# shurizzle/cake

Hardware: AMD Instinct MI355X
Metric: decode_tokens_per_sec (higher is better)
Workload: dtype bf16; 1 GPU; model=Llama-3-8B, global_batch=1, seq_len=1097, prompt_len=32, parallelism=single, decode=greedy, repeat_penalty 1.10 last_n 128

## Files before the change

### cake_amd/csrc/kernels/gemv_kernel.h

```cpp
#pragma once
#include <type_traits>

#include "common.h"

namespace cake {

constexpr int kGemvThreads = 256;
constexpr int kGemvWaves = kGemvThreads / 64;
constexpr int kGemvMaxBlocks = 1024;

typedef float f32x2_t __attribute__((ext_vector_type(2)));

struct GemvTune { int U, PF, MB; };
enum GemvKind { kQkv = 0, kSwiglu = 1, kX16 = 2, kNormF32 = 3, kX16S = 4, kNumKinds = 5 };
extern GemvTune g_tune[4][kNumKinds];


template <class T>
__device__ __forceinline__ const T* pick3(const T* q, const T* k, const T* v, int kind) {
  const ptrdiff_t dk = k - q, dv = v - q;
  return q + (kind == 0 ? 0 : (kind == 1 ? dk : dv));
}

struct PlainRows {
  struct Rows { const uint4 *a, *b; };
  struct Chunk { uint4 a, b; };
  template <bool NT> static __device__ __forceinline__ Chunk load(const Rows& r, int c) {
    if constexpr (NT) return {ld_nt16(r.a + c), ld_nt16(r.b + c)};
    else return {r.a[c], r.b[c]};
  }
  template <int LOG2> static int prefetch_if_filled(int pf, int K) {
    return (K >> LOG2) >= 64 * pf ? pf : 0;
  }
};

template <int DT, bool XF32>
__device__ __forceinline__ void load_x8(const void* xs, int chunk, float* o) {
  if constexpr (XF32) {
    const float4* p = reinterpret_cast<const float4*>(xs) + chunk * 2;
    const float4 a = p[0], b = p[1];
    o[0] = a.x; o[1] = a.y; o[2] = a.z; o[3] = a.w;
    o[4] = b.x; o[5] = b.y; o[6] = b.z; o[7] = b.w;
  } else {
    unpack8<DT>(reinterpret_cast<const uint4*>(xs)[chunk], o);
  }
}

struct W16 : PlainRows {
  static constexpr int kFmt = 0, kKinds = kNumKinds, kLog2 = 3, kPad32 = 1, kPad16 = 1;
  static constexpr int kU[3] = {2, 4, 8}, kPF[2] = {8, 4};
  static constexpr bool kStrict = false, kRowScale = false;
  static __device__ __forceinline__ int perm32(int i) { return i; }
  static __device__ __forceinline__ int perm16(int i) { return i; }
  static int prefetch(int pf, int K) { return prefetch_if_filled<kLog2>(pf, K); }
  using Acc = float;
  static __device__ __forceinline__ Acc zero() { return 0.f; }
  static __device__ __forceinline__ float total(Acc a) { return a; }
  struct Mat { const uint16_t* w; };
  static __device__ __forceinline__ Mat pick(const Mat& q, const Mat& k, const Mat& v, int kind) {
    return {pick3(q.w, k.w, v.w, kind)};
  }
  static __device__ __forceinline__ Rows rows(const Mat& ma, size_t ra, const Mat& mb, size_t rb,
                                              int K) {
    return {reinterpret_cast<const uint4*>(ma.w + ra * K),
            reinterpret_cast<const uint4*>(mb.w + rb * K)};
  }
  template <int DT, bool XF32>
  static __device__ __forceinline__ void fma(const void* xs, int chunk, const Chunk& v, Acc& acc_a,
                                             Acc& acc_b) {
    float xv[8], fa[8], fb[8];
    load_x8<DT, XF32>(xs, chunk, xv);
    unpack8<DT>(v.a, fa);
    unpack8<DT>(v.b, fb);
#pragma unroll
    for (int e = 0; e < 8; ++e) {
      acc_a = fmaf(fa[e], xv[e], acc_a);
      acc_b = fmaf(fb[e], xv[e], acc_b);
    }
  }
};

template <class F, class = void> struct HasRawRows : std::false_type {};
template <class F>
struct HasRawRows<F, std::void_t<decltype(F::kRawRows)>> : std::bool_constant<F::kRawRows> {};

template <class F, class = void> struct Bf16Only : std::false_type {};
template <class F>
struct Bf16Only<F, std::void_t<decltype(F::kBf16Only)>> : std::bool_constant<F::kBf16Only> {};

template <class F, int U, class = void> struct X16Waves : std::integral_constant<int, 1> {};
template <class F, int U>
struct X16Waves<F, U, std::void_t<decltype(F::x16_waves(U))>>
    : std::integral_constant<int, F::x16_waves(U)> {};

template <class F>
__device__ __forceinline__ float row_scale(const typename F::Mat& m, size_t row) {
  if constexpr (F::kRowScale) return m.scale[row];
  else return 1.f;
}
template <class F>
__device__ __forceinline__ float descale(float d, bool first, float s0, const typename F::Mat& m,
                                         size_t row) {
  if constexpr (F::kRowScale) return d * (first ? s0 : m.scale[row]);
  else return d;
}


template <class F, int DT>
__device__ __forceinline__ void stage_rmsnorm(const float* __restrict__ x,
                                              const uint16_t* __restrict__ w,
                                              float eps, int K, float* xs) {
  __shared__ float red[16];
  float ss = 0.f;
  for (int i = threadIdx.x * 4; i < K; i += kGemvThreads * 4) {
    const float4 v = *reinterpret_cast<const float4*>(x + i);
    *reinterpret_cast<float4*>(xs + F::perm32(i)) = v;
    ss += v.x * v.x + v.y * v.y + v.z * v.z + v.w * v.w;
  }
  ss = block_sum(ss, red);
  const float r = rsqrtf(ss / (float)K + eps);
  for (int i = threadIdx.x * 4; i < K; i += kGemvThreads * 4) {
    float4 v = *reinterpret_cast<float4*>(xs + F::perm32(i));
    const uint2 wv = *reinterpret_cast<const uint2*>(w + i);
    v.x *= r * to_f32<DT>((uint16_t)(wv.x & 0xffff));
    v.y *= r * to_f32<DT>((uint16_t)(wv.x >> 16));
    v.z *= r * to_f32<DT>((uint16_t)(wv.y & 0xffff));
    v.w *= r * to_f32<DT>((uint16_t)(wv.y >> 16));
    *reinterpret_cast<float4*>(xs + F::perm32(i)) = v;
  }
  __syncthreads();
}

template <class F>
__device__ __forceinline__ void stage_plain16(const uint16_t* __restrict__ x, int K,
                                              uint16_t* xs) {
  for (int i = threadIdx.x * 8; i < K; i += kGemvThreads * 8)
    *reinterpret_cast<uint4*>(xs + F::perm16(i)) = *reinterpret_cast<const uint4*>(x + i);
  __syncthreads();
}

template <class F, int DT, int NX> struct NormPre {
  float4 x[NX];
  uint2 w[NX];
  __device__ __forceinline__ void load(const float* __restrict__ xg, const uint16_t* __restrict__ wg,
                                       int K) {
#pragma unroll
    for (int j = 0; j < NX; ++j) {
      const int i = (j * kGemvThreads + threadIdx.x) * 4;
      x[j] = i < K ? *reinterpret_cast<const float4*>(xg + i) : make_float4(0.f, 0.f, 0.f, 0.f);
      w[j] = i < K ? *reinterpret_cast<const uint2*>(wg + i) : make_uint2(0u, 0u);
    }
  }
  __device__ __forceinline__ void finish(float eps, int K, float* xs) {
    __shared__ float red[16];
    float ss = 0.f;
#pragma unroll
    for (int j = 0; j < NX; ++j) ss += x[j].x * x[j].x + x[j].y * x[j].y + x[j].z * x[j].z + x[j].w * x[j].w;
    ss = block_sum(ss, red);
    const float r = rsqrtf(ss / (float)K + eps);
#pragma unroll
    for (int j = 0; j < NX; ++j) {
      const int i = (j * kGemvThreads + threadIdx.x) * 4;
      float4 v = x[j];
      v.x *= r * to_f32<DT>((uint16_t)(w[j].x & 0xffff));
      v.y *= r * to_f32<DT>((uint16_t)(w[j].x >> 16));
      v.z *= r * to_f32<DT>((uint16_t)(w[j].y & 0xffff));
      v.w *= r * to_f32<DT>((uint16_t)(w[j].y >> 16));
      if (i < K) *reinterpret_cast<float4*>(xs + F::perm32(i)) = v;
    }
    __syncthreads();
  }
};

template <class F, int NX> struct Plain16Pre {
  uint4 v[NX];
  __device__ __forceinline__ void load(const uint16_t* __restrict__ xg, int K) {
#pragma unroll
    for (int j = 0; j < NX; ++j) {
      const int i = (j * kGemvThreads + threadIdx.x) * 8;
      v[j] = i < K ? *reinterpret_cast<const uint4*>(xg + i) : make_uint4(0u, 0u, 0u, 0u);
    }
  }
  __device__ __forceinline__ void finish(int K, uint16_t* xs) {
#pragma unroll
    for (int j = 0; j < NX; ++j) {
      const int i = (j * kGemvThreads + threadIdx.x) * 8;
      if (i < K) *reinterpret_cast<uint4*>(xs + F::perm16(i)) = v[j];
    }
    __syncthreads();
  }
};


template <class F, int DT, bool XF32, int U>
__device__ __forceinline__ void dot_range(const typename F::Rows& r, const void* xs, int nch,
                                          int c_start, typename F::Acc& acc_a,
                                          typename F::Acc& acc_b) {
  const int lane = threadIdx.x & 63;
  const int full = c_start + ((nch - c_start) / (64 * U)) * (64 * U);
  for (int c0 = c_start; c0 < full; c0 += 64 * U) {
    typename F::Chunk v[U];
#pragma unroll
    for (int u = 0; u < U; ++u) v[u] = F::template load<true>(r, c0 + u * 64 + lane);
#pragma unroll
    for (int u = 0; u < U; ++u) F::template fma<DT, XF32>(xs, c0 + u * 64 + lane, v[u], acc_a, acc_b);
  }
  for (int c = full + lane; c < nch; c += 64)
    F::template fma<DT, XF32>(xs, c, F::template load<false>(r, c), acc_a, acc_b);
}

template <class F, int PFC, bool RAW = HasRawRows<F>::value> struct Regs {
  typename F::Chunk c[PFC > 0 ? PFC : 1];
};
template <class F, int PFC> struct Regs<F, PFC, true> {
  typename F::Chunk c[PFC > 0 ? PFC : 1];
  typename F::Rows r;
};

template <class F, int PFC>
__device__ __forceinline__ void prefetch_rows(const typename F::Rows& r, Regs<F, PFC>& g) {
  if constexpr (PFC > 0) {
    const int lane = threadIdx.x & 63;
#pragma unroll
    for (int c = 0; c < PFC; ++c) g.c[c] = F::template load<true>(r, c * 64 + lane);
  }
}

template <class F, int PFC>
__device__ __forceinline__ void keep_rows(const typename F::Rows& r, Regs<F, PFC>& g) {
  if constexpr (HasRawRows<F>::value) g.r = r;
}

template <class F, int DT, bool XF32, int U, int PFC, class Map, class Epi>
__device__ __forceinline__ void run_pairs_raw(const Map& map, const Epi& epi, const void* xs, int K,
                                              int npairs, int p0, int stride,
                                              const Regs<F, PFC>& pre) {
  const int nch = K >> F::kLog2;
  auto raw_dots = [&](const typename F::Rows& r, float& aa, float& ab) {
    dot_range<W16, DT, XF32, 4>(F::raw_rows(r, K), xs, K >> W16::kLog2, 0, aa, ab);
  };
  auto clamped = [&](int q) { return map(q < npairs ? q : npairs - 1); };
  int p = p0;
  typename F::Rows rn;
  if constexpr (PFC > 0) {
    const typename F::Rows r = pre.r;
    rn = clamped(p + stride);
    const int lane = threadIdx.x & 63;
    if (F::is_raw(r)) {
      float aa = 0.f, ab = 0.f;
      raw_dots(r, aa, ab);
      const float sa = wave_sum(aa), sb = wave_sum(ab);
      if (p < npairs) epi(p, sa, sb);
    } else {
      typename F::Acc aa = F::zero(), ab = F::zero();
#pragma unroll
      for (int c = 0; c < PFC; ++c) F::template fma<DT, XF32>(xs, c * 64 + lane, pre.c[c], aa, ab);
      dot_range<F, DT, XF32, U>(r, xs, nch, PFC * 64, aa, ab);
      const float sa = wave_sum(F::total(aa)), sb = wave_sum(F::total(ab));
      if (p < npairs) epi(p, sa, sb);
    }
    p += stride;
  } else {
    rn = clamped(p);
  }
  for (; p < npairs; p += stride) {
    const typename F::Rows r = rn;
    rn = clamped(p + stride);
    if (F::is_raw(r)) {
      float aa = 0.f, ab = 0.f;
      raw_dots(r, aa, ab);
      epi(p, wave_sum(aa), wave_sum(ab));
      continue;
    }
    typename F::Acc aa = F::zero(), ab = F::zero();
    dot_range<F, DT, XF32, U>(r, xs, nch, 0, aa, ab);
    epi(p, wave_sum(F::total(aa)), wave_sum(F::total(ab)));
  }
}

template <class F, int DT, bool XF32, int U, int PFC, class Map, class Epi>
__device__ __forceinline__ void run_pairs(const Map& map, const Epi& epi, const void* xs, int K,
                                          int npairs, int p0, int stride,
                                          const Regs<F, PFC>& pre) {
  if constexpr (HasRawRows<F>::value) {
    run_pairs_raw<F, DT, XF32, U, PFC>(map, epi, xs, K, npairs, p0, stride, pre);
    return;
  }
  const int nch = K >> F::kLog2;
  int p = p0;
  if constexpr (PFC > 0) {
    const typename F::Rows r = map(p < npairs ? p : npairs - 1);
    const int lane = threadIdx.x & 63;
    typename F::Acc aa = F::zero(), ab = F::zero();
#pragma unroll
    for (int c = 0; c < PFC; ++c) F::template fma<DT, XF32>(xs, c * 64 + lane, pre.c[c], aa, ab);
    dot_range<F, DT, XF32, U>(r, xs, nch, PFC * 64, aa, ab);
    const float sa = wave_sum(F::total(aa)), sb = wave_sum(F::total(ab));
    if (p < npairs) epi(p, sa, sb);
    p += stride;
  }
  for (; p < npairs; p += stride) {
    const typename F::Rows r = map(p);
    typename F::Acc aa = F::zero(), ab = F::zero();
    dot_range<F, DT, XF32, U>(r, xs, nch, 0, aa, ab);
    epi(p, wave_sum(F::total(aa)), wave_sum(F::total(ab)));
  }
}

template <class F> struct QkvArgs {
  const float* resid;
  const uint16_t* norm_w;
  float eps;
  typename F::Mat q, k, v;
  int K, nh, nkv, hd;
  const float* inv_freq;
  const int* pos;
  float* q_out;
  uint16_t* kcache;
  uint16_t* vcache;
  int S;
  int kv_fmt;
};

struct QkvPair {
  int kind, head, i;
  size_t ra;
};

__device__ __forceinline__ QkvPair qkv_pair(int p, int half, int nh, int nqk, int hd) {
  const int slot = p / half;
  const bool isq = slot < nh, isk = !isq && slot < nqk;
  QkvPair r;
  r.kind = isq ? 0 : (isk ? 1 : 2);
  r.head = slot - (isq ? 0 : (isk ? nh : nqk));
  r.i = p - slot * half;
  r.ra = (size_t)r.head * hd + r.i;
  return r;
}

template <class F, int DT, int U, int PFC, int NX>
__global__ __launch_bounds__(kGemvThreads) void qkv_rope_kernel(QkvArgs<F> a) {
  extern __shared__ float xs[];
  const int half = a.hd >> 1;
  const int npairs = (a.nh + 2 * a.nkv) * half;
  const int wave = threadIdx.x >> 6, lane = threadIdx.x & 63;
  const int p0 = blockIdx.x * kGemvWaves + wave;
  const int nh = a.nh, nqk = a.nh + a.nkv, hd = a.hd, K = a.K;
  auto map = [&](int p) {
    const QkvPair r = qkv_pair(p, half, nh, nqk, hd);
    const typename F::Mat m = F::pick(a.q, a.k, a.v, r.kind);
    return F::rows(m, r.ra, m, r.ra + half, K);
  };
  Regs<F, PFC> pre;
  NormPre<F, DT, NX> xp;
  const int pc = p0 < npairs ? p0 : npairs - 1;
  const typename F::Rows r0 = map(pc);
  keep_rows<F, PFC>(r0, pre);
  if constexpr (NX > 0) xp.load(a.resid, a.norm_w, a.K);
  __builtin_amdgcn_sched_barrier(0);
  if (NX > 0 || (PFC > 0 && p0 < npairs)) prefetch_rows<F, PFC>(r0, pre);
  const QkvPair rc = qkv_pair(pc, half, nh, nqk, hd);
  const float f0 = a.inv_freq[rc.i];
  const typename F::Mat mc = F::pick(a.q, a.k, a.v, rc.kind);
  const float s0a = row_scale<F>(mc, rc.ra), s0b = row_scale<F>(mc, rc.ra + half);
  __builtin_amdgcn_sched_barrier(0);
  if constexpr (NX > 0) xp.finish(a.eps, a.K, xs);
  else stage_rmsnorm<F, DT>(a.resid, a.norm_w, a.eps, a.K, xs);
  const int pos = *a.pos;
  auto epi = [&](int p, float da, float db) {
    if (lane != 0) return;
    const QkvPair r = qkv_pair(p, half, nh, nqk, hd);
    const typename F::Mat m = F::pick(a.q, a.k, a.v, r.kind);
    if constexpr (F::kRowScale) {
      float sa = s0a, sb = s0b;
      if (p != p0) { sa = m.scale[r.ra]; sb = m.scale[r.ra + half]; }
      da *= sa;
      db *= sb;
    }
    float oa = da, ob = db;
    if (r.kind < 2) {
      float s, c;
      sincosf((float)pos * (p == p0 ? f0 : a.inv_freq[r.i]), &s, &c);
      oa = da * c - db * s;
      ob = da * s + db * c;
    }
    if (r.kind == 0) {
      a.q_out[r.ra] = oa;
      a.q_out[r.ra + half] = ob;
    } else {
      uint16_t* cache = r.kind == 1 ? a.kcache : a.vcache;
      const size_t off = ((size_t)r.head * a.S + pos) * a.hd + r.i;
      kv_store_pair<DT>(cache, off, half, oa, ob, a.kv_fmt);
    }
  };
  run_pairs<F, DT, true, U, PFC>(map, epi, xs, a.K, npairs, p0, gridDim.x * kGemvWaves, pre);
}

template <class F, int DT, int U, int PFC, int NX>
__global__ __launch_bounds__(kGemvThreads) void swiglu_kernel(
    const float* __restrict__ resid, const uint16_t* __restrict__ norm_w, float eps,
    const typename F::Mat wg, const typename F::Mat wu, int K, int I,
    uint16_t* __restrict__ act) {
  extern __shared__ float xs[];
  const int wave = threadIdx.x >> 6, lane = threadIdx.x & 63;
  const int j0 = blockIdx.x * kGemvWaves + wave;
  auto map = [&](int j) { return F::rows(wg, (size_t)j, wu, (size_t)j, K); };
  Regs<F, PFC> pre;
  NormPre<F, DT, NX> xp;
  const int jp = j0 < I ? j0 : I - 1;
  const typename F::Rows r0 = map(jp);
  keep_rows<F, PFC>(r0, pre);
  if constexpr (NX > 0) xp.load(resid, norm_w, K);
  __builtin_amdgcn_sched_barrier(0);
  if (NX > 0 || (PFC > 0 && j0 < I)) prefetch_rows<F, PFC>(r0, pre);
  const float s0g = row_scale<F>(wg, jp), s0u = row_scale<F>(wu, jp);
  __builtin_amdgcn_sched_barrier(0);
  if constexpr (NX > 0) xp.finish(eps, K, xs);
  else stage_rmsnorm<F, DT>(resid, norm_w, eps, K, xs);
  auto epi = [&](int j, float g, float u) {
    if (lane != 0) return;
    g = descale<F>(g, j == j0, s0g, wg, j);
    u = descale<F>(u, j == j0, s0u, wu, j);
    act[j] = from_f32<DT>(silu(g) * u);
  };
  run_pairs<F, DT, true, U, PFC>(map, epi, xs, K, I, j0, gridDim.x * kGemvWaves, pre);
}

template <class F, int DT, int U, int PFC, int NX, bool ACCUM>
__global__ __launch_bounds__(kGemvThreads) __attribute__((amdgpu_waves_per_eu(X16Waves<F, U>::value)))
void gemv_x16_kernel(
    const uint16_t* __restrict__ x, const typename F::Mat w, int K, int N,
    float* __restrict__ out) {
  extern __shared__ float smem[];
  uint16_t* xs = reinterpret_cast<uint16_t*>(smem);
  const int wave = threadIdx.x >> 6, lane = threadIdx.x & 63;
  const int npairs = (N + 1) >> 1;
  const int p0 = blockIdx.x * kGemvWaves + wave;
  auto map = [&](int p) { return F::rows(w, (size_t)(2 * p), w, (size_t)min(2 * p + 1, N - 1), K); };
  Regs<F, PFC> pre;
  Plain16Pre<F, NX> xp;
  const int pc = p0 < npairs ? p0 : npairs - 1;
  const typename F::Rows r0 = map(pc);
  keep_rows<F, PFC>(r0, pre);
  if constexpr (NX > 0) xp.load(x, K);
  __builtin_amdgcn_sched_barrier(0);
  if (NX > 0 || (PFC > 0 && p0 < npairs)) prefetch_rows<F, PFC>(r0, pre);
  const float s0a = row_scale<F>(w, 2 * pc), s0b = row_scale<F>(w, min(2 * pc + 1, N - 1));
  float r0a = 0.f, r0b = 0.f;
  if constexpr (ACCUM) {
    r0a = out[2 * pc];
    r0b = out[min(2 * pc + 1, N - 1)];
  }
  __builtin_amdgcn_sched_barrier(0);
  if constexpr (NX > 0) xp.finish(K, xs);
  else stage_plain16<F>(x, K, xs);
  auto epi = [&](int p, float da, float db) {
    if (lane != 0) return;
    const int ra = 2 * p, rb = 2 * p + 1;
    da = descale<F>(da, p == p0, s0a, w, ra);
    if (ACCUM) out[ra] = da + (p == p0 ? r0a : out[ra]); else out[ra] = da;
    if (rb < N) {
      db = descale<F>(db, p == p0, s0b, w, rb);
      if (ACCUM) out[rb] = db + (p == p0 ? r0b : out[rb]); else out[rb] = db;
    }
  };
  run_pairs<F, DT, false, U, PFC>(map, epi, xs, K, npairs, p0, gridDim.x * kGemvWaves, pre);
}

struct HeadSel {
  const int* hist;
  const int* hist_len;
  int last_n;
  float penalty;
  unsigned long long* slot;
  unsigned int* ticket;
  int* tok;
  int* hist_w;
  int* hist_len_w;
  int* pos;
  int max_hist;
  const uint16_t* embed;
  float* emb_out;
  int H;
};

__device__ __forceinline__ unsigned int ordered_key(float f) {
  const unsigned int u = __float_as_uint(f);
  return (u & 0x80000000u) ? ~u : (u | 0x80000000u);
}

__device__ __forceinline__ void head_sel_window(const HeadSel& hs, int hlen, int lane, int* win) {
  const int n = min(hs.last_n, hlen), start = hlen - n;
#pragma unroll
  for (int j = 0; j < 4; ++j) win[j] = j * 64 + lane < n ? hs.hist[start + j * 64 + lane] : -1;
}

__device__ __forceinline__ void head_sel_pair(const HeadSel& hs, const int* win, int ra, int rb,
                                              int N, float& da, float& db,
                                              unsigned long long& best) {
  if (hs.penalty != 1.f) {
    const bool ia = win[0] == ra || win[1] == ra || win[2] == ra || win[3] == ra;
    const bool ib = win[0] == rb || win[1] == rb || win[2] == rb || win[3] == rb;
    if (__builtin_amdgcn_ballot_w64(ia) != 0ull) da = da >= 0.f ? da / hs.penalty : da * hs.penalty;
    if (__builtin_amdgcn_ballot_w64(ib) != 0ull) db = db >= 0.f ? db / hs.penalty : db * hs.penalty;
  }
  const unsigned long long ka =
      ((unsigned long long)ordered_key(da) << 32) | (0xffffffffu - (unsigned int)ra);
  best = ka > best ? ka : best;
  if (rb < N) {
    const unsigned long long kb =
        ((unsigned long long)ordered_key(db) << 32) | (0xffffffffu - (unsigned int)rb);
    best = kb > best ? kb : best;
  }
}

template <int DT>
__device__ __forceinline__ void head_sel_tail(const HeadSel& hs, unsigned long long best,
                                              void* lds) {
  const int wave = threadIdx.x >> 6, lane = threadIdx.x & 63;
  unsigned long long* red = reinterpret_cast<unsigned long long*>(lds);
  int& is_last = reinterpret_cast<int*>(lds)[2 * kGemvWaves];
  int& sel_tok = reinterpret_cast<int*>(lds)[2 * kGemvWaves + 1];
  __syncthreads();
  if (lane == 0) red[wave] = best;
  __syncthreads();
  if (threadIdx.x == 0) {
    unsigned long long b = red[0];
#pragma unroll
    for (int i = 1; i < kGemvWaves; ++i) b = red[i] > b ? red[i] : b;
    const unsigned long long old =
        __hip_atomic_fetch_max(hs.slot, b, __ATOMIC_RELAXED, __HIP_MEMORY_SCOPE_AGENT);
    asm volatile("s_waitcnt vmcnt(0)" ::"v"((unsigned int)old) : "memory");
    const unsigned int t =
        __hip_atomic_fetch_add(hs.ticket, 1u, __ATOMIC_RELAXED, __HIP_MEMORY_SCOPE_AGENT);
    is_last = t == gridDim.x - 1;
  }
  __syncthreads();
  if (is_last) {
    if (threadIdx.x == 0) {
      const unsigned long long key =
          __hip_atomic_fetch_max(hs.slot, 0ull, __ATOMIC_RELAXED, __HIP_MEMORY_SCOPE_AGENT);
      const int t = (int)(0xffffffffu - (unsigned int)(key & 0xffffffffull));
      *hs.tok = t;
      const int len = *hs.hist_len_w;
      if (len < hs.max_hist) { hs.hist_w[len] = t; *hs.hist_len_w = len + 1; }
      *hs.pos += 1;
      __hip_atomic_store(hs.slot, 0ull, __ATOMIC_RELAXED, __HIP_MEMORY_SCOPE_AGENT);
      __hip_atomic_store(hs.ticket, 0u, __ATOMIC_RELAXED, __HIP_MEMORY_SCOPE_AGENT);
      sel_tok = t;
    }
    if (hs.embed != nullptr) {
      __syncthreads();
      const uint16_t* row = hs.embed + (size_t)sel_tok * hs.H;
      for (int i = threadIdx.x * 8; i < hs.H; i += kGemvThreads * 8) {
        float f[8];
        unpack8<DT>(*reinterpret_cast<const uint4*>(row + i), f);
        *reinterpret_cast<float4*>(hs.emb_out + i) = make_float4(f[0], f[1], f[2], f[3]);
        *reinterpret_cast<float4*>(hs.emb_out + i + 4) = make_float4(f[4], f[5], f[6], f[7]);
      }
    }
  }
}

template <class F, int DT, int U, int PFC, int NX, bool SEL>
__global__ __launch_bounds__(kGemvThreads) void gemv_norm_f32_kernel(
    const float* __restrict__ resid, const uint16_t* __restrict__ norm_w, float eps,
    const typename F::Mat w, int K, int N, float* __restrict__ out, HeadSel hs) {
  extern __shared__ float xs[];
  const int wave = threadIdx.x >> 6, lane = threadIdx.x & 63;
  const int npairs = (N + 1) >> 1;
  const int p0 = blockIdx.x * kGemvWaves + wave;
  auto map = [&](int p) { return F::rows(w, (size_t)(2 * p), w, (size_t)min(2 * p + 1, N - 1), K); };
  int hlen = 0;
  if constexpr (SEL) hlen = hs.penalty != 1.f ? *hs.hist_len : 0;
  Regs<F, PFC> pre;
  NormPre<F, DT, NX> xp;
  const int pc = p0 < npairs ? p0 : npairs - 1;
  const typename F::Rows r0 = map(pc);
  keep_rows<F, PFC>(r0, pre);
  if constexpr (NX > 0) xp.load(resid, norm_w, K);
  __builtin_amdgcn_sched_barrier(0);
  if (NX > 0 || (PFC > 0 && p0 < npairs)) prefetch_rows<F, PFC>(r0, pre);
  const float s0a = row_scale<F>(w, 2 * pc), s0b = row_scale<F>(w, min(2 * pc + 1, N - 1));
  __builtin_amdgcn_sched_barrier(0);
  if constexpr (NX > 0) xp.finish(eps, K, xs);
  else stage_rmsnorm<F, DT>(resid, norm_w, eps, K, xs);
  int win[4] = {-1, -1, -1, -1};
  if constexpr (SEL) head_sel_window(hs, hlen, lane, win);
  unsigned long long best = 0ull;
  auto epi = [&](int p, float da, float db) {
    const int ra = 2 * p, rb = 2 * p + 1;
    da = descale<F>(da, p == p0, s0a, w, ra);
    db = descale<F>(db, p == p0, s0b, w, min(rb, N - 1));
    if constexpr (SEL) head_sel_pair(hs, win, ra, rb, N, da, db, best);
    if (lane != 0) return;
    out[ra] = da;
    if (rb < N) out[rb] = db;
  };
  run_pairs<F, DT, true, U, PFC>(map, epi, xs, K, npairs, p0, gridDim.x * kGemvWaves, pre);
  if constexpr (SEL) head_sel_tail<DT>(hs, best, xs);
}

static inline int grid_for(int npairs, int max_blocks) {
  int g = (npairs + kGemvWaves - 1) / kGemvWaves;
  return g < max_blocks ? g : max_blocks;
}

}

using namespace cake;


#define DISPATCH_DT(dt, ...)                       \
  do {                                             \
    if ((dt) == kBF16) { constexpr int DT = kBF16; __VA_ARGS__; } \
    else if ((dt) == kF16) { constexpr int DT = kF16; __VA_ARGS__; } \
    else return (int)hipErrorInvalidValue;         \
  } while (0)
#define DISPATCH_DT_F(F, dt, ...)                  \
  do {                                             \
    if constexpr (Bf16Only<F>::value) {            \
      if ((dt) == kBF16) { constexpr int DT = kBF16; __VA_ARGS__; } \
      else return (int)hipErrorInvalidValue;       \
    } else DISPATCH_DT(dt, __VA_ARGS__);           \
  } while (0)

#define CAKE_TUNE_U(F, PFCV, ...)                                                              \
  if (t.U == F::kU[0]) { constexpr int U = F::kU[0]; constexpr int PF = PFCV; __VA_ARGS__; }      \
  else if (t.U == F::kU[1]) { constexpr int U = F::kU[1]; constexpr int PF = PFCV; __VA_ARGS__; } \
  else { constexpr int U = F::kU[2]; constexpr int PF = PFCV; __VA_ARGS__; }
#define DISPATCH_TUNE(F, t, K, ...)                                                  \
  do {                                                                               \
    const int pfc_ = F::prefetch((t).PF, K);                                         \
    if (pfc_ == F::kPF[0]) { CAKE_TUNE_U(F, F::kPF[0], __VA_ARGS__) }                \
    else if (pfc_ == F::kPF[1]) { CAKE_TUNE_U(F, F::kPF[1], __VA_ARGS__) }           \
    else { CAKE_TUNE_U(F, 0, __VA_ARGS__) }                                          \
  } while (0)
#define CAKE_NX_NORM(K, ...)                                                         \
  if constexpr (PF > 0) {                                                            \
    if ((K) <= 4096) { constexpr int NX = 4; __VA_ARGS__; }                          \
    else if ((K) <= 8192) { constexpr int NX = 8; __VA_ARGS__; }                     \
    else { constexpr int NX = 0; __VA_ARGS__; }                                      \
  } else { constexpr int NX = 0; __VA_ARGS__; }
#define CAKE_NX_X16(K, ...)                                                          \
  if constexpr (PF > 0) {                                                            \
    if ((K) <= 2048) { constexpr int NX = 1; __VA_ARGS__; }                          \
    else if ((K) <= 4096) { constexpr int NX = 2; __VA_ARGS__; }                     \
    else if ((K) <= 8192) { constexpr int NX = 4; __VA_ARGS__; }                     \
    else if ((K) <= 14336) { constexpr int NX = 7; __VA_ARGS__; }                    \
    else if ((K) <= 28672) { constexpr int NX = 14; __VA_ARGS__; }                   \
    else { constexpr int NX = 0; __VA_ARGS__; }                                      \
  } else { constexpr int NX = 0; __VA_ARGS__; }

template <class F> static inline bool bad_shape(int K, int n) {
  return K % (1 << F::kLog2) != 0 || (F::kStrict && (K < (1 << F::kLog2) || n < 1));
}
template <class F> static inline size_t x32_lds_bytes(int K) {
  return (size_t)((K + F::kPad32 - 1) / F::kPad32 * F::kPad32) * sizeof(float);
}
template <class F> static inline size_t x16_lds_bytes(int K) {
  return (size_t)((K + F::kPad16 - 1) / F::kPad16 * F::kPad16) * sizeof(uint16_t);
}

template <class F> static int gemv_set_tuning(int kind, int U, int prefetch, int max_blocks) {
  if (kind < 0 || kind >= F::kKinds || (U != F::kU[0] && U != F::kU[1] && U != F::kU[2]) ||
      max_blocks < 1 || (prefetch != 0 && prefetch != F::kPF[0] && prefetch != F::kPF[1]))
    return (int)hipErrorInvalidValue;
  g_tune[F::kFmt][kind] = GemvTune{U, prefetch, max_blocks};
  return 0;
}

template <class F> static int gemv_get_tuning(int kind, int* out3) {
  if (kind < 0 || kind >= F::kKinds || !out3) return (int)hipErrorInvalidValue;
  const GemvTune t = g_tune[F::kFmt][kind];
  out3[0] = t.U;
  out3[1] = t.PF;
  out3[2] = t.MB;
  return 0;
}

template <class F> static int launch_qkv(int dt, const QkvArgs<F>& a, hipStream_t st) {
  if (bad_shape<F>(a.K, a.nh < a.nkv ? a.nh : a.nkv) || a.hd % 2 || a.kv_fmt < 0 || a.kv_fmt > 2)
    return (int)hipErrorInvalidValue;
  const int K = a.K, npairs = (a.nh + 2 * a.nkv) * (a.hd / 2);
  const size_t lds = x32_lds_bytes<F>(K);
  const GemvTune t = g_tune[F::kFmt][kQkv];
  DISPATCH_DT_F(F, dt, DISPATCH_TUNE(F, t, K, CAKE_NX_NORM(K, hipLaunchKernelGGL((qkv_rope_kernel<F, DT, U, PF, NX>),
                                                         dim3(grid_for(npairs, t.MB)),
                                                         dim3(kGemvThreads), lds, st, a))));
  return (int)hipGetLastError();
}

template <class F>
static int launch_swiglu(int dt, const float* resid, const void* norm_w, float eps,
                         typename F::Mat wg, typename F::Mat wu, int K, int I, void* act,
                         hipStream_t st) {
  if (bad_shape<F>(K, I)) return (int)hipErrorInvalidValue;
  const size_t lds = x32_lds_bytes<F>(K);
  const GemvTune t = g_tune[F::kFmt][kSwiglu];
  const int mb = t.MB > (I + 27) / 28 ? t.MB : (I + 27) / 28;
  DISPATCH_DT_F(F, dt, DISPATCH_TUNE(F, t, K, CAKE_NX_NORM(K, hipLaunchKernelGGL((swiglu_kernel<F, DT, U, PF, NX>),
                                                         dim3(grid_for(I, mb)), dim3(kGemvThreads),
                                                         lds, st, resid, (const uint16_t*)norm_w, eps,
                                                         wg, wu, K, I, (uint16_t*)act))));
  return (int)hipGetLastError();
}

template <class F>
static int launch_x16(int dt, const void* x, typename F::Mat w, int K, int N, float* out,
                      int accumulate, hipStream_t st) {
  if (bad_shape<F>(K, N)) return (int)hipErrorInvalidValue;
  const size_t lds = x16_lds_bytes<F>(K);
  const GemvTune t = g_tune[F::kFmt][F::kKinds > kX16S && K <= 8192 ? kX16S : kX16];
  const int g = grid_for((N + 1) / 2, t.MB);
  if (accumulate) {
    DISPATCH_DT_F(F, dt, DISPATCH_TUNE(F, t, K, CAKE_NX_X16(K, hipLaunchKernelGGL((gemv_x16_kernel<F, DT, U, PF, NX, true>),
                                                          dim3(g), dim3(kGemvThreads), lds, st,
                                                          (const uint16_t*)x, w, K, N, out))));
  } else {
    DISPATCH_DT_F(F, dt, DISPATCH_TUNE(F, t, K, CAKE_NX_X16(K, hipLaunchKernelGGL((gemv_x16_kernel<F, DT, U, PF, NX, false>),
                                                          dim3(g), dim3(kGemvThreads), lds, st,
                                                          (const uint16_t*)x, w, K, N, out))));
  }
  return (int)hipGetLastError();
}

template <class F, bool SEL>
static int launch_norm_f32(int dt, const float* resid, const void* norm_w, float eps,
                           typename F::Mat w, int K, int N, float* out, const HeadSel& hs,
                           hipStream_t st) {
  if (bad_shape<F>(K, N)) return (int)hipErrorInvalidValue;
  const size_t lds = SEL && x32_lds_bytes<F>(K) < 64 ? 64 : x32_lds_bytes<F>(K);
  const GemvTune t = g_tune[F::kFmt][kNormF32];
  DISPATCH_DT_F(F, dt, DISPATCH_TUNE(F, t, K, CAKE_NX_NORM(K, hipLaunchKernelGGL((gemv_norm_f32_kernel<F, DT, U, PF, NX, SEL>),
                                                         dim3(grid_for((N + 1) / 2, t.MB)),
                                                         dim3(kGemvThreads), lds, st, resid,
                                                         (const uint16_t*)norm_w, eps, w, K, N,
                                                         out, hs))));
  return (int)hipGetLastError();
}

template <class F>
static int launch_head_select(int dt, const float* resid, const void* norm_w, float eps,
                              typename F::Mat w, int K, int N, float* out, int* hist,
                              int* hist_len, int last_n, float penalty, unsigned long long* slot,
                              unsigned int* ticket, int* tok, int* pos, int max_hist,
                              const void* embed, float* emb_out, hipStream_t st) {
  if (last_n < 0 || last_n > kHeadSelectMaxLastN || !(penalty > 0.f) || slot == nullptr ||
      ticket == nullptr || (embed != nullptr && emb_out == nullptr))
    return (int)hipErrorInvalidValue;
  const HeadSel hs{hist, hist_len, last_n, penalty, slot, ticket, tok, hist, hist_len, pos,
                   max_hist, (const uint16_t*)embed, emb_out, K};
  return launch_norm_f32<F, true>(dt, resid, norm_w, eps, w, K, N, out, hs, st);
}
```

### cake_amd/csrc/kernels/gemv_p13_kernel.h

```cpp
#pragma once
#include "gemv_kernel.h"

namespace cake {

constexpr int kP13Tile = 2048;
constexpr int kP13TileBytes = 3328;
enum PackKind { kPackAdjacent = 0, kPackHeadHalves = 1, kPackGateUp = 2 };

__host__ __device__ inline int p13_partner(int kind, int r, int N, int hd) {
  if (kind == kPackHeadHalves) return r % hd < hd / 2 ? r + hd / 2 : r - hd / 2;
  if (kind == kPackGateUp) return r < N / 2 ? r + N / 2 : r - N / 2;
  return (r ^ 1) < N ? (r ^ 1) : r;
}

__device__ __forceinline__ uint32_t p13_base4(int hdr) {
  return (uint32_t)(hdr & 0x7f) * 0x01010101u;
}

__device__ __forceinline__ void p13_high(uint32_t code, uint32_t sgn, int j, uint32_t base4,
                                         uint32_t& hia, uint32_t& hib) {
  const uint32_t ca = code & 0x0f0f0f0fu, cb = (code >> 4) & 0x0f0f0f0fu;
  const uint32_t ta = (ca + 0x7f7f7f7fu) & 0x80808080u, tb = (cb + 0x7f7f7f7fu) & 0x80808080u;
  const uint32_t ha = ca + ((ta - (ta >> 7)) & base4), hb = cb + ((tb - (tb >> 7)) & base4);
  const uint32_t sa = sgn << (7 - 2 * j), sb = sgn << (6 - 2 * j);
  hia = (ha & 0x7f7f7f7fu) | (sa & 0x80808080u);
  hib = (hb & 0x7f7f7f7fu) | (sb & 0x80808080u);
}

__device__ __forceinline__ uint4 p13_decode8(uint32_t lo0, uint32_t lo1, uint32_t code,
                                             uint32_t sgn, int j, uint32_t base4) {
  uint32_t hia, hib;
  p13_high(code, sgn, j, base4, hia, hib);
  uint4 o;
  o.x = __builtin_amdgcn_perm(hia, lo0, 0x05010400u);
  o.y = __builtin_amdgcn_perm(hia, lo0, 0x07030602u);
  o.z = __builtin_amdgcn_perm(hib, lo1, 0x05010400u);
  o.w = __builtin_amdgcn_perm(hib, lo1, 0x07030602u);
  return o;
}

__device__ __forceinline__ void p13_decode8f(uint32_t lo0, uint32_t lo1, uint32_t code,
                                             uint32_t sgn, int j, uint32_t base4, float* o) {
  uint32_t hia, hib;
  p13_high(code, sgn, j, base4, hia, hib);
  o[0] = __uint_as_float(__builtin_amdgcn_perm(hia, lo0, 0x04000c0cu));
  o[1] = __uint_as_float(__builtin_amdgcn_perm(hia, lo0, 0x05010c0cu));
  o[2] = __uint_as_float(__builtin_amdgcn_perm(hia, lo0, 0x06020c0cu));
  o[3] = __uint_as_float(__builtin_amdgcn_perm(hia, lo0, 0x07030c0cu));
  o[4] = __uint_as_float(__builtin_amdgcn_perm(hib, lo1, 0x04000c0cu));
  o[5] = __uint_as_float(__builtin_amdgcn_perm(hib, lo1, 0x05010c0cu));
  o[6] = __uint_as_float(__builtin_amdgcn_perm(hib, lo1, 0x06020c0cu));
  o[7] = __uint_as_float(__builtin_amdgcn_perm(hib, lo1, 0x07030c0cu));
}

__device__ __forceinline__ uint32_t ld_nt4(const uint32_t* p) { return __builtin_nontemporal_load(p); }

struct P13 {
  static constexpr int kFmt = 3, kKinds = kNumKinds, kLog2 = 5, kPad32 = 1, kPad16 = 1;
  static constexpr int kU[3] = {1, 2, 3}, kPF[2] = {2, 1};
  static constexpr bool kStrict = true, kRowScale = false, kRawRows = true, kBf16Only = true;
  static constexpr int x16_waves(int U) { return U == 1 ? 3 : 1; }
  static __device__ __forceinline__ int perm32(int i) { return i; }
  static __device__ __forceinline__ int perm16(int i) { return i; }
  static int prefetch(int pf, int K) { return PlainRows::prefetch_if_filled<kLog2>(pf, K); }
  using Acc = float;
  static __device__ __forceinline__ Acc zero() { return 0.f; }
  static __device__ __forceinline__ float total(Acc a) { return a; }
  struct Mat {
    const uint8_t* planes;
    const int* hdr;
    const uint16_t* raw;
  };
  static __device__ __forceinline__ Mat pick(const Mat& q, const Mat& k, const Mat& v, int kind) {
    return {pick3(q.planes, k.planes, v.planes, kind), pick3(q.hdr, k.hdr, v.hdr, kind),
            pick3(q.raw, k.raw, v.raw, kind)};
  }
  struct Rows {
    const uint8_t *a, *b;
    int ha, hb;
    const uint16_t *rawa, *rawb;
  };
  static __device__ __forceinline__ Rows rows(const Mat& ma, size_t ra, const Mat& mb, size_t rb,
                                              int K) {
    const size_t rowb = (size_t)(K / kP13Tile) * kP13TileBytes;
    return {ma.planes + ra * rowb, mb.planes + rb * rowb, ma.hdr[ra], mb.hdr[rb], ma.raw, mb.raw};
  }
  static __device__ __forceinline__ bool is_raw(const Rows& r) {
    return (__builtin_amdgcn_readfirstlane(r.ha | r.hb) >> 8) != 0;
  }
  static __device__ __forceinline__ PlainRows::Rows raw_rows(const Rows& r, int K) {
    const int sa = __builtin_amdgcn_readfirstlane(r.ha) >> 8;
    const int sb = __builtin_amdgcn_readfirstlane(r.hb) >> 8;
    return {reinterpret_cast<const uint4*>(r.rawa + (size_t)(sa - 1) * K),
            reinterpret_cast<const uint4*>(r.rawb + (size_t)(sb - 1) * K)};
  }
  struct Chunk {
    uint4 la0, la1, ca, lb0, lb1, cb;
    uint32_t sa, sb;
    int ha, hb;
  };
  template <bool NT> static __device__ __forceinline__ Chunk load(const Rows& r, int c) {
    const size_t t = (size_t)(c >> 6) * kP13TileBytes;
    const int l = c & 63;
    const uint4* pa = reinterpret_cast<const uint4*>(r.a + t) + l;
    const uint4* pb = reinterpret_cast<const uint4*>(r.b + t) + l;
    const uint32_t* qa = reinterpret_cast<const uint32_t*>(r.a + t + 3072) + l;
    const uint32_t* qb = reinterpret_cast<const uint32_t*>(r.b + t + 3072) + l;
    Chunk v;
    if constexpr (NT) {
      v.la0 = ld_nt16(pa); v.la1 = ld_nt16(pa + 64); v.ca = ld_nt16(pa + 128); v.sa = ld_nt4(qa);
      v.lb0 = ld_nt16(pb); v.lb1 = ld_nt16(pb + 64); v.cb = ld_nt16(pb + 128); v.sb = ld_nt4(qb);
    } else {
      v.la0 = pa[0]; v.la1 = pa[64]; v.ca = pa[128]; v.sa = *qa;
      v.lb0 = pb[0]; v.lb1 = pb[64]; v.cb = pb[128]; v.sb = *qb;
    }
    v.ha = r.ha;
    v.hb = r.hb;
    return v;
  }
  template <int DT, bool XF32>
  static __device__ __forceinline__ void fma(const void* xs, int chunk, const Chunk& v, Acc& acc_a,
                                             Acc& acc_b) {
    if constexpr (DT == kBF16) {
      const int c16 = ((chunk >> 6) << 8) + (chunk & 63);
      const uint32_t la[8] = {v.la0.x, v.la0.y, v.la0.z, v.la0.w, v.la1.x, v.la1.y, v.la1.z, v.la1.w};
      const uint32_t lb[8] = {v.lb0.x, v.lb0.y, v.lb0.z, v.lb0.w, v.lb1.x, v.lb1.y, v.lb1.z, v.lb1.w};
      const uint32_t ca[4] = {v.ca.x, v.ca.y, v.ca.z, v.ca.w};
      const uint32_t cb[4] = {v.cb.x, v.cb.y, v.cb.z, v.cb.w};
      const uint32_t base_a = p13_base4(v.ha), base_b = p13_base4(v.hb);
#pragma unroll
      for (int j = 0; j < 4; ++j) {
        float xv[8], fa[8], fb[8];
        load_x8<DT, XF32>(xs, c16 + j * 64, xv);
        p13_decode8f(la[2 * j], la[2 * j + 1], ca[j], v.sa, j, base_a, fa);
        p13_decode8f(lb[2 * j], lb[2 * j + 1], cb[j], v.sb, j, base_b, fb);
#pragma unroll
        for (int e = 0; e < 8; ++e) {
          acc_a = fmaf(fa[e], xv[e], acc_a);
          acc_b = fmaf(fb[e], xv[e], acc_b);
        }
      }
    }
  }
};

static inline bool p13_bad(int dt, int K, const void* planes, const void* hdr) {
  return dt != kBF16 || K < kP13Tile || K % kP13Tile != 0 || planes == nullptr || hdr == nullptr;
}

}
```

Measured before the change: 391.2 tokens/s.

## Software-pipeline P13 GEMV chunk loads across row pairs with a rolling register ring

Replaces the per-pair loop in the raw-row GEMV path with a flat, chunk-level software pipeline. A ring of D prefetched chunks is refilled continuously across pair boundaries, so loads for the next row pair are in flight while the current one is finishing. Row headers are now loaded per chunk instead of when rows are mapped, which moves the raw-row check onto the chunk. The x16 wave count is also fixed at 2. The ring adds register pressure and control complexity, and the raw fallback path now re-maps the row at pair end.

```diff
diff --git a/cake_amd/csrc/kernels/gemv_kernel.h b/cake_amd/csrc/kernels/gemv_kernel.h
--- a/cake_amd/csrc/kernels/gemv_kernel.h
+++ b/cake_amd/csrc/kernels/gemv_kernel.h
@@ -235,46 +235,72 @@
 __device__ __forceinline__ void run_pairs_raw(const Map& map, const Epi& epi, const void* xs, int K,
                                               int npairs, int p0, int stride,
                                               const Regs<F, PFC>& pre) {
-  const int nch = K >> F::kLog2;
-  auto raw_dots = [&](const typename F::Rows& r, float& aa, float& ab) {
-    dot_range<W16, DT, XF32, 4>(F::raw_rows(r, K), xs, K >> W16::kLog2, 0, aa, ab);
+  constexpr int D = U > PFC ? U : PFC;
+  const int nt = K >> (F::kLog2 + 6);
+  const int lane = threadIdx.x & 63;
+  const int T = p0 < npairs ? ((npairs - 1 - p0) / stride + 1) * nt : 0;
+  int qi = p0, ki = PFC;
+  typename F::Rows ri = pre.r;
+  auto issue = [&](typename F::Chunk& set) {
+    if (ki == nt) {
+      ki = 0;
+      qi += stride;
+      ri = map(qi);
+    }
+    set = F::template load<true>(ri, ki * 64 + lane);
+    ++ki;
   };
-  auto clamped = [&](int q) { return map(q < npairs ? q : npairs - 1); };
-  int p = p0;
-  typename F::Rows rn;
-  if constexpr (PFC > 0) {
-    const typename F::Rows r = pre.r;
-    rn = clamped(p + stride);
-    const int lane = threadIdx.x & 63;
-    if (F::is_raw(r)) {
-      float aa = 0.f, ab = 0.f;
-      raw_dots(r, aa, ab);
-      const float sa = wave_sum(aa), sb = wave_sum(ab);
-      if (p < npairs) epi(p, sa, sb);
-    } else {
-      typename F::Acc aa = F::zero(), ab = F::zero();
-#pragma unroll
-      for (int c = 0; c < PFC; ++c) F::template fma<DT, XF32>(xs, c * 64 + lane, pre.c[c], aa, ab);
-      dot_range<F, DT, XF32, U>(r, xs, nch, PFC * 64, aa, ab);
-      const float sa = wave_sum(F::total(aa)), sb = wave_sum(F::total(ab));
-      if (p < npairs) epi(p, sa, sb);
-    }
-    p += stride;
+  int pc = p0, kc = 0;
+  typename F::Acc aa = F::zero(), ab = F::zero();
+  auto decode = [&](const typename F::Chunk& v) {
+    const bool raw = F::is_raw(v);
+    if (!raw) F::template fma<DT, XF32>(xs, kc * 64 + lane, v, aa, ab);
+    return raw;
+  };
+  auto pair_end = [&](const typename F::Chunk& v, bool raw) {
+    if (++kc < nt) return;
+    if (raw) {
+      aa = F::zero();
+      ab = F::zero();
+      dot_range<W16, DT, XF32, 4>(F::raw_rows(map(pc), v, K), xs, K >> W16::kLog2, 0, aa, ab);
+    }
+    epi(pc, wave_sum(F::total(aa)), wave_sum(F::total(ab)));
+    aa = F::zero();
+    ab = F::zero();
+    kc = 0;
+    pc += stride;
+  };
+  typename F::Chunk set[D];
+#pragma unroll
+  for (int s = 0; s < PFC; ++s) set[s] = pre.c[s];
+  int t = 0;
+  if (T >= 2 * D) {
+#pragma unroll
+    for (int s = PFC; s < D; ++s) issue(set[s]);
+    for (; T - t >= 2 * D; t += D) {
+#pragma unroll
+      for (int s = 0; s < D; ++s) {
+        const typename F::Chunk v = set[s];
+        const bool raw = decode(v);
+        issue(set[s]);
+        pair_end(v, raw);
+      }
+    }
   } else {
-    rn = clamped(p);
-  }
-  for (; p < npairs; p += stride) {
-    const typename F::Rows r = rn;
-    rn = clamped(p + stride);
-    if (F::is_raw(r)) {
-      float aa = 0.f, ab = 0.f;
-      raw_dots(r, aa, ab);
-      epi(p, wave_sum(aa), wave_sum(ab));
-      continue;
-    }
-    typename F::Acc aa = F::zero(), ab = F::zero();
-    dot_range<F, DT, XF32, U>(r, xs, nch, 0, aa, ab);
-    epi(p, wave_sum(F::total(aa)), wave_sum(F::total(ab)));
+#pragma unroll
+    for (int s = PFC; s < D; ++s)
+      if (s < T) issue(set[s]);
+  }
+#pragma unroll
+  for (int r = 0; r < 2; ++r) {
+#pragma unroll
+    for (int s = 0; s < D; ++s, ++t) {
+      if (t >= T) continue;
+      const typename F::Chunk v = set[s];
+      const bool raw = decode(v);
+      if (r == 0 && t + D < T) issue(set[s]);
+      pair_end(v, raw);
+    }
   }
 }
 
diff --git a/cake_amd/csrc/kernels/gemv_p13_kernel.h b/cake_amd/csrc/kernels/gemv_p13_kernel.h
--- a/cake_amd/csrc/kernels/gemv_p13_kernel.h
+++ b/cake_amd/csrc/kernels/gemv_p13_kernel.h
@@ -59,7 +59,7 @@
   static constexpr int kFmt = 3, kKinds = kNumKinds, kLog2 = 5, kPad32 = 1, kPad16 = 1;
   static constexpr int kU[3] = {1, 2, 3}, kPF[2] = {2, 1};
   static constexpr bool kStrict = true, kRowScale = false, kRawRows = true, kBf16Only = true;
-  static constexpr int x16_waves(int U) { return U == 1 ? 3 : 1; }
+  static constexpr int x16_waves(int) { return 2; }
   static __device__ __forceinline__ int perm32(int i) { return i; }
   static __device__ __forceinline__ int perm16(int i) { return i; }
   static int prefetch(int pf, int K) { return PlainRows::prefetch_if_filled<kLog2>(pf, K); }
@@ -77,28 +77,28 @@
   }
   struct Rows {
     const uint8_t *a, *b;
-    int ha, hb;
+    const int *ha, *hb;
     const uint16_t *rawa, *rawb;
   };
   static __device__ __forceinline__ Rows rows(const Mat& ma, size_t ra, const Mat& mb, size_t rb,
                                               int K) {
     const size_t rowb = (size_t)(K / kP13Tile) * kP13TileBytes;
-    return {ma.planes + ra * rowb, mb.planes + rb * rowb, ma.hdr[ra], mb.hdr[rb], ma.raw, mb.raw};
-  }
-  static __device__ __forceinline__ bool is_raw(const Rows& r) {
-    return (__builtin_amdgcn_readfirstlane(r.ha | r.hb) >> 8) != 0;
-  }
-  static __device__ __forceinline__ PlainRows::Rows raw_rows(const Rows& r, int K) {
-    const int sa = __builtin_amdgcn_readfirstlane(r.ha) >> 8;
-    const int sb = __builtin_amdgcn_readfirstlane(r.hb) >> 8;
-    return {reinterpret_cast<const uint4*>(r.rawa + (size_t)(sa - 1) * K),
-            reinterpret_cast<const uint4*>(r.rawb + (size_t)(sb - 1) * K)};
+    return {ma.planes + ra * rowb, mb.planes + rb * rowb, ma.hdr + ra, mb.hdr + rb, ma.raw, mb.raw};
   }
   struct Chunk {
     uint4 la0, la1, ca, lb0, lb1, cb;
     uint32_t sa, sb;
     int ha, hb;
   };
+  static __device__ __forceinline__ bool is_raw(const Chunk& v) {
+    return (__builtin_amdgcn_readfirstlane(v.ha | v.hb) >> 8) != 0;
+  }
+  static __device__ __forceinline__ PlainRows::Rows raw_rows(const Rows& r, const Chunk& v, int K) {
+    const int sa = __builtin_amdgcn_readfirstlane(v.ha) >> 8;
+    const int sb = __builtin_amdgcn_readfirstlane(v.hb) >> 8;
+    return {reinterpret_cast<const uint4*>(r.rawa + (size_t)(sa - 1) * K),
+            reinterpret_cast<const uint4*>(r.rawb + (size_t)(sb - 1) * K)};
+  }
   template <bool NT> static __device__ __forceinline__ Chunk load(const Rows& r, int c) {
     const size_t t = (size_t)(c >> 6) * kP13TileBytes;
     const int l = c & 63;
@@ -107,6 +107,8 @@
     const uint32_t* qa = reinterpret_cast<const uint32_t*>(r.a + t + 3072) + l;
     const uint32_t* qb = reinterpret_cast<const uint32_t*>(r.b + t + 3072) + l;
     Chunk v;
+    v.ha = *r.ha;
+    v.hb = *r.hb;
     if constexpr (NT) {
       v.la0 = ld_nt16(pa); v.la1 = ld_nt16(pa + 64); v.ca = ld_nt16(pa + 128); v.sa = ld_nt4(qa);
       v.lb0 = ld_nt16(pb); v.lb1 = ld_nt16(pb + 64); v.cb = ld_nt16(pb + 128); v.sb = ld_nt4(qb);
@@ -114,8 +116,6 @@
       v.la0 = pa[0]; v.la1 = pa[64]; v.ca = pa[128]; v.sa = *qa;
       v.lb0 = pb[0]; v.lb1 = pb[64]; v.cb = pb[128]; v.sb = *qb;
     }
-    v.ha = r.ha;
-    v.hb = r.hb;
     return v;
   }
   template <int DT, bool XF32>
```

Measured after the change: 392.0 tokens/s (median of 5 runs). About the same (+0.2%).
